# url-kaist/Quatro

Measured on NVIDIA H100. Metric: registrations/sec (64-ring pair), higher is better.
Workload: dtype f32 (front end, match, graph filter) / f64 (graph boundary, GNC, COTE)

## Files before the change

### quatro_b200/csrc/clique.cu

```cuda
#include "handle.cuh"

namespace qb {

__device__ __forceinline__ int warp_max(int v) { return __reduce_max_sync(0xffffffffu, v); }
__device__ __forceinline__ int warp_sum(int v) { return __reduce_add_sync(0xffffffffu, v); }

__device__ void warp_bucket_sort(const unsigned short* __restrict__ key, int n, int maxkey, int* __restrict__ bin,
                                 unsigned short* __restrict__ pos, unsigned short* __restrict__ vert) {
  const int lane = lane_id();
  for (int d = lane; d <= maxkey + 1; d += 32) bin[d] = 0;
  __syncwarp();
  for (int v = lane; v < n; v += 32) atomicAdd(&bin[key[v]], 1);
  __syncwarp();
  int carry = 0;
  for (int base = 0; base <= maxkey + 1; base += 32) {
    const int d = base + lane;
    const int c = d <= maxkey + 1 ? bin[d] : 0;
    int tot;
    const int ex = warp_excl_scan(c, &tot);
    if (d <= maxkey + 1) bin[d] = carry + ex;
    carry += tot;
  }
  __syncwarp();
  for (int base = 0; base < n; base += 32) {
// ... 26 lines not shown
constexpr int kRing = 16;

__device__ __forceinline__ void cp_async4(void* smem_dst, const void* gsrc) {
  const unsigned d = (unsigned)__cvta_generic_to_shared(smem_dst);
  asm volatile("cp.async.ca.shared.global [%0], [%1], 4;" ::"r"(d), "l"(gsrc) : "memory");
}
__device__ __forceinline__ void cp_async_commit() { asm volatile("cp.async.commit_group;" ::: "memory"); }
template <int N>
__device__ __forceinline__ void cp_async_wait() { asm volatile("cp.async.wait_group %0;" ::"n"(N) : "memory"); }

constexpr int kKcWarps = 4;

__device__ __forceinline__ void kcore_apply_moves(const unsigned short* __restrict__ nbl, int cnt, int dv, int* __restrict__ bin,
                                                  unsigned short* __restrict__ deg, unsigned short* __restrict__ pos,
                                                  unsigned short* __restrict__ vert, unsigned short* __restrict__ mrk,
                                                  uint32_t* __restrict__ above_own, uint32_t* __restrict__ add_next, bool classes) {
  const int lane = lane_id();
  const unsigned lt = (1u << lane) - 1u;
  for (int c0 = 0; c0 < cnt; c0 += 32) {
    const int e = c0 + lane;
    const bool act = e < cnt;
    const int u = act ? nbl[e] : 0;
    const int du = act ? deg[u] : -1 - lane;
    const unsigned grp = __match_any_sync(0xffffffffu, du);
    const int rank = __popc(grp & lt), m = __popc(grp);
    int b0 = 0, pu = 0;
    if (act) {
      b0 = bin[du];
      pu = pos[u];
      mrk[u] = (unsigned short)(rank + 1);
    }
    __syncwarp();
    int y = -1;
    if (act && pu >= b0 + m) {
      int curk = rank;
      for (;;) {
        y = vert[b0 + curk];
        const int r = mrk[y];
        if (r == 0) break;
        curk = r - 1;
      }
    }
    __syncwarp();
    if (act) {
      vert[b0 + rank] = (unsigned short)u; pos[u] = (unsigned short)(b0 + rank);
      if (y >= 0) { vert[pu] = (unsigned short)y; pos[y] = (unsigned short)pu; }
      mrk[u] = 0;
      deg[u] = (unsigned short)(du - 1);
      const uint32_t bit = 1u << (u & 31);
      if (classes) {
        atomicAnd(&above_own[u >> 5], ~bit);
        if (du - 1 > dv) atomicOr(&add_next[u >> 5], bit);
      } else if (du - 1 == dv) {
        atomicAnd(&above_own[u >> 5], ~bit);
      }
      if (rank == 0) bin[du] = b0 + m;
    }
    __syncwarp();
  }
}

template <int WPL>
__device__ __forceinline__ int kcore_expand(const uint32_t (&w)[WPL], int w0, unsigned short* __restrict__ nbl) {
  int c = 0;
#pragma unroll
  for (int k = 0; k < WPL; ++k) c += __popc(w[k]);
  int cnt;
  int off = warp_excl_scan(c, &cnt);
  if (cnt != 0) {
#pragma unroll
    for (int k = 0; k < WPL; ++k) {
      uint32_t x = w[k];
      const int basebit = (w0 + k) * 32;
      while (x) {
        const int b = __ffs(x) - 1;
        x &= x - 1;
        nbl[off++] = (unsigned short)(basebit + b);
      }
    }
  }
  return cnt;
}

template <int WPL, bool kWs>
__global__ void __maxnreg__(168) kcore_kernel(const uint32_t* __restrict__ adj, const int* __restrict__ deg_in,
                                                              const int* __restrict__ n_corr, const PairSolve* __restrict__ solve, int Lc, int W,
                                                              int Ls, int row_words, unsigned char* __restrict__ ws, int* __restrict__ kcore,
                                                              int* __restrict__ korder, int* __restrict__ rank_of, int* __restrict__ by_rank,
                                                              int* __restrict__ kbin, int* __restrict__ max_core_out) {
  constexpr int NW = kKcWarps, AW = 32 * WPL;
  extern __shared__ __align__(16) unsigned char smem_raw[];
  __shared__ int ring_tag[kRing];

  const int pair = blockIdx.x, tid = threadIdx.x, lane = tid & 31, warp = tid >> 5;
  if (solve[pair].mode == QB200_INLIER_NONE) return;
  const int L = n_corr[pair];
  if ((L > Ls) != kWs) return;
  constexpr bool in_smem = !kWs;
  const int Lv = in_smem ? Ls : Lc;
  int* bin = in_smem ? reinterpret_cast<int*>(smem_raw)
                     : reinterpret_cast<int*>(ws + (size_t)pair * kcore_ws_bytes(Lc));
  uint32_t* above = in_smem ? reinterpret_cast<uint32_t*>(bin + Ls + 2)
                            : reinterpret_cast<uint32_t*>(smem_raw);
  uint32_t* add = above + NW * AW;
  uint32_t* rows = add + 2 * NW * AW;
  unsigned short* deg = in_smem ? reinterpret_cast<unsigned short*>(rows + row_words) : reinterpret_cast<unsigned short*>(bin + Lc + 2);
  unsigned short* pos = deg + Lv;
  unsigned short* vert = pos + Lv;
  unsigned short* mrk = vert + Lv;
  unsigned short* nbl_all = mrk + Lv;
  int* __restrict__ kc = kcore + (size_t)pair * (Lc + 2);
  int* __restrict__ ko = korder + (size_t)pair * (Lc + 2);
  int* __restrict__ ro = rank_of + (size_t)pair * (Lc + 2);
  int* __restrict__ br = by_rank + (size_t)pair * (Lc + 2);
  int* __restrict__ kb = kbin + (size_t)pair * (Lc + 2);
  if (L <= 0) {
    if (tid == 0) max_core_out[pair] = 0;
    return;
  }
  const uint32_t* __restrict__ G = adj + (size_t)pair * Lc * W;
  const int nbw = (L + 31) >> 5;
  const int nwl = (nbw + 31) >> 5;
  const bool cached = in_smem && (long long)L * nbw <= (long long)row_words;
  const int rs = in_smem ? Ls / 32 : W;
  const int w0 = lane * nwl;
  unsigned short* nbl = nbl_all + (size_t)warp * Lv;

  int md = 0;
  for (int v = tid; v < L; v += NW * 32) {
    const int d = deg_in[(size_t)pair * Lc + v];
    deg[v] = (unsigned short)d;
    mrk[v] = 0;
    md = max(md, d);
  }
  if (cached)
    for (int idx = tid; idx < L * nbw; idx += NW * 32) rows[idx] = G[(size_t)(idx / nbw) * W + (idx % nbw)];
  for (int wd = tid; wd < 3 * NW * AW; wd += NW * 32) above[wd] = 0u;
  __shared__ int s_md[NW];
  md = warp_max(md);
  if (lane == 0) s_md[warp] = md;
  __syncthreads();
  md = max(max(s_md[0], s_md[1]), max(s_md[2], s_md[3]));
  if (warp == 0) warp_bucket_sort(deg, L, md, bin, pos, vert);
  __syncthreads();
  for (int v = tid; v < L; v += NW * 32) {
    const int c = cached ? 0 : (int)deg[v] % NW;
    atomicOr(&above[c * AW + (v >> 5)], 1u << (v & 31));
  }
  __syncthreads();

  int cur = -1;
  if (cached) {
    if (warp != 0) return;
    for (int i = 0; i < L; ++i) {
      const int v = vert[i];
      const int dv = deg[v];
      if (dv > cur) {
        const int end = bin[dv + 1];
        for (int p = i + lane; p < end; p += 32) {
          const int x = vert[p];
          atomicAnd(&above[x >> 5], ~(1u << (x & 31)));
        }
        cur = dv;
        __syncwarp();
      }
      uint32_t w[WPL];
#pragma unroll
      for (int k = 0; k < WPL; ++k) w[k] = (k < nwl && w0 + k < nbw) ? (rows[v * nbw + w0 + k] & above[w0 + k]) : 0u;
      const int cnt = kcore_expand<WPL>(w, w0, nbl);
      if (cnt == 0) continue;
      __syncwarp();
      kcore_apply_moves(nbl, cnt, dv, bin, deg, pos, vert, mrk, above, above, false);
    }
  } else {
    uint32_t* above_w = above + warp * AW;
    const int lower = (warp + NW - 1) % NW;
    auto fetch = [&](int p) {
      if (p < L) {
        const int x = vert[p], sl = p % kRing;
        if (lane == 0) ring_tag[sl] = x;
#pragma unroll
        for (int k = 0; k < WPL; ++k)
          if (k < nwl && w0 + k < nbw) cp_async4(rows + sl * rs + w0 + k, G + (size_t)x * W + w0 + k);
      }
      cp_async_commit();
    };
    if (warp == 0) {
      for (int p = 0; p < kRing - 1; ++p) fetch(p);
      cp_async_wait<kRing - 2>();
    }
    __syncthreads();
    for (int i = 0; i < L; ++i) {
      const int v = vert[i];
      const int dv = deg[v];
      const int par = i & 1;
      if (warp == 0) fetch(i + kRing - 1);
      uint32_t* add_in = add + ((par ^ 1) * NW + warp) * AW;
      uint32_t w[WPL];
      const int sl = i % kRing;
      const bool hit = ring_tag[sl] == v;
#pragma unroll
      for (int k = 0; k < WPL; ++k) {
        w[k] = 0u;
        if (k < nwl && w0 + k < nbw) {
          const uint32_t a = add_in[w0 + k];
          if (a) { above_w[w0 + k] |= a; add_in[w0 + k] = 0u; }
          w[k] = hit ? rows[sl * rs + w0 + k] : G[(size_t)v * W + w0 + k];
        }
      }
      __syncwarp();
      if (dv > cur) {
        if (dv % NW == warp) {
          const int end = bin[dv + 1];
          for (int p = i + lane; p < end; p += 32) {
            const int x = vert[p];
            atomicAnd(&above_w[x >> 5], ~(1u << (x & 31)));
          }
          __syncwarp();
        }
        cur = dv;
      }
#pragma unroll
      for (int k = 0; k < WPL; ++k) w[k] = (k < nwl && w0 + k < nbw) ? (w[k] & above_w[w0 + k]) : 0u;
      const int cnt = kcore_expand<WPL>(w, w0, nbl);
      if (cnt != 0) {
        __syncwarp();
        kcore_apply_moves(nbl, cnt, dv, bin, deg, pos, vert, mrk, above_w, add + (par * NW + lower) * AW, true);
      }
      if (warp == 0) cp_async_wait<kRing - 2>();
      __syncthreads();
    }
    if (warp == 0) cp_async_wait<0>();
    if (warp != 0) return;
  }
  __syncwarp();
  const int max_core = deg[vert[L - 1]];
  for (int v = lane; v < L; v += 32) {
    kc[v] = (int)deg[v] + 1;
    ko[v] = vert[v];
  }
  if (lane == 0) max_core_out[pair] = max_core;
  __syncwarp();
  warp_bucket_sort(deg, L, max_core, bin, pos, vert);
  for (int v = lane; v < L; v += 32) {
    ro[v] = pos[v];
    br[v] = vert[v];
  }
  for (int d = lane; d <= max_core + 1; d += 32) kb[d] = bin[d];
}

__global__ void __launch_bounds__(256) permute_adj_kernel(const uint32_t* __restrict__ adj, const int* __restrict__ n_corr, int Lc, int W,
                                                          const PairSolve* __restrict__ solve, const int* __restrict__ rank_of,
                                                          uint32_t* __restrict__ adjp) {
  extern __shared__ uint32_t rows[];
  const int pair = blockIdx.y;
  if (solve[pair].mode == QB200_INLIER_NONE) return;
  const int L = n_corr[pair];
  const int wib = threadIdx.x >> 5, lane = lane_id();
  const int v = blockIdx.x * 8 + wib;
  if (v >= L) return;
  uint32_t* row = rows + wib * W;
  const int nb = (L + 31) >> 5;
  for (int w = lane; w < nb; w += 32) row[w] = 0;
  __syncwarp();
  const int* __restrict__ ro = rank_of + (size_t)pair * (Lc + 2);
  const uint32_t* __restrict__ src = adj + ((size_t)pair * Lc + v) * W;
  for (int w = lane; w < nb; w += 32) {
    uint32_t x = src[w];
    while (x) {
      const int b = __ffs(x) - 1;
      x &= x - 1;
      const int r = ro[w * 32 + b];
      atomicOr(&row[r >> 5], 1u << (r & 31));
    }
  }
  __syncwarp();
  uint32_t* __restrict__ dst = adjp + ((size_t)pair * Lc + ro[v]) * W;
  for (int w = lane; w < nb; w += 32) dst[w] = row[w];
}

template <int WPL>
__device__ __forceinline__ int clique_descent(const uint32_t* __restrict__ rows, int stride, int nbw, int rv, int thr, int mc,
                                              unsigned short* __restrict__ chain) {
  const int lane = lane_id();
  uint32_t P[WPL];
  int psize = 0;
#pragma unroll
  for (int k = 0; k < WPL; ++k) {
    const int wi = lane + 32 * k;
    uint32_t x = wi < nbw ? rows[(size_t)rv * stride + wi] : 0u;
    const int lo = wi * 32;
    if (thr >= lo + 32) x = 0;
    else if (thr > lo) x &= ~0u << (thr - lo);
    P[k] = x;
    psize += __popc(x);
  }
  psize = warp_sum(psize);
  if (psize <= mc) return 0;
  int sz = 1;
  for (;;) {
    int top = -1;
#pragma unroll
    for (int k = 0; k < WPL; ++k)
      if (P[k]) top = max(top, (lane + 32 * k) * 32 + 31 - __clz(P[k]));
    top = warp_max(top);
    if (top < 0) break;
    if (lane == 0) chain[sz - 1] = (unsigned short)top;
    ++sz;
#pragma unroll
    for (int k = 0; k < WPL; ++k) {
      const int wi = lane + 32 * k;
      P[k] &= wi < nbw ? rows[(size_t)top * stride + wi] : 0u;
    }
  }
  return sz;
}

__global__ void __launch_bounds__(kCliqueWarps * 32) clique_cta_kernel(const uint32_t* __restrict__ adjp, const int* __restrict__ n_corr, int Lc, int W,
                                                                       int Ls, unsigned short* __restrict__ chain_ws,
                                                                       const int* __restrict__ kcore, const int* __restrict__ korder,
                                                                       const int* __restrict__ rank_of, const int* __restrict__ by_rank,
                                                                       const int* __restrict__ kbin, const int* __restrict__ max_core_in,
                                                                       const PairSolve* __restrict__ solve, int cache_words, int* __restrict__ clique,
                                                                       int* __restrict__ n_clique) {
  constexpr int NT = kCliqueWarps * 32;
  extern __shared__ __align__(16) unsigned char smem_raw[];
  uint32_t* idbits = reinterpret_cast<uint32_t*>(smem_raw + (size_t)kCliqueWarps * Ls * sizeof(unsigned short));
  uint32_t* cache = idbits + W;
  __shared__ int s_sz[kCliqueWarps];
  __shared__ int s_scan[33];
  const int pair = blockIdx.x, tid = threadIdx.x, lane = tid & 31, warp = tid >> 5;
// ... 196 lines not shown
      const int a = max(thr, lo), b = min(L, lo + 32);
      if (wi < nbw && a < b) x = (b - lo >= 32 ? ~0u : ((1u << (b - lo)) - 1u)) & (~0u << (a - lo));
      P[k] = x;
      if (wi < nbw) SP[wi] = x;
    }
  }
  int used = exact_colour_sort<WPL>(rows, stride, nbw, P, best, LP, kExactPool);
  bool truncated = used < 0;
  int depth = truncated ? -1 : 0;
  if (lane == 0 && !truncated) { lb[0] = 0; ln[0] = used; }
  __syncwarp();
  long long nodes = 0;
  bool improved = false;
  while (depth >= 0) {
    const int n_here = ln[depth];
    if (n_here == 0) { --depth; continue; }
    const int begin = lb[depth];
    const uint32_t e = LP[begin + n_here - 1];
    __syncwarp();
    if (lane == 0) ln[depth] = n_here - 1;
    const int v = (int)(e & 0xFFFFu), col = (int)(e >> 16);
    if (depth + col <= best) {
      if (lane == 0) ln[depth] = 0;
      __syncwarp();
      continue;
    }
    if (lane == 0) C[depth] = (unsigned short)v;
    uint32_t* __restrict__ Pl = SP + (size_t)depth * W;
    int cnt = 0;
#pragma unroll
    for (int k = 0; k < WPL; ++k) {
      const int wi = lane + 32 * k;
      uint32_t x = 0u;
      if (wi < nbw) {
        const uint32_t pw = Pl[wi];
        x = pw & rows[(size_t)v * stride + wi];
        if (wi == (v >> 5)) Pl[wi] = pw & ~(1u << (v & 31));
      }
      P[k] = x;
      cnt += __popc(x);
    }
    cnt = __reduce_add_sync(0xffffffffu, cnt);
    __syncwarp();
    if (cnt == 0) {
      if (depth + 1 > best) {
        best = depth + 1;
        improved = true;
        for (int t = lane; t <= depth; t += 32) out[t] = br[C[t]];
        __syncwarp();
        if (best >= ub) break;
      }
      continue;
    }
    if (depth + 1 + cnt <= best) continue;
    if (++nodes > node_limit || depth + 1 >= kExactDepth) { truncated = true; break; }
    const int nbegin = begin + n_here - 1;
    uint32_t* __restrict__ Pn = SP + (size_t)(depth + 1) * W;
#pragma unroll
    for (int k = 0; k < WPL; ++k) {
      const int wi = lane + 32 * k;
      if (wi < nbw) Pn[wi] = P[k];
    }
    const int nl = exact_colour_sort<WPL>(rows, stride, nbw, P, best - (depth + 1), LP + nbegin, kExactPool - nbegin);
    if (nl < 0) { truncated = true; break; }
    if (lane == 0) { lb[depth + 1] = nbegin; ln[depth + 1] = nl; }
    __syncwarp();
    ++depth;
  }
  __syncwarp();
  if (improved) {
    for (int t = lane; t < best; t += 32) {
      const int x = out[t];
      int r = 0;
      for (int u = 0; u < best; ++u) r += out[u] < x ? 1 : 0;
      lb[r] = x;
    }
    __syncwarp();
    for (int t = lane; t < best; t += 32) out[t] = lb[t];
    if (lane == 0) n_clique[pair] = best;
  }
  if (lane == 0 && truncated) flags[pair] |= QB200_FLAG_CLIQUE_TRUNCATED;
}

constexpr size_t kKcoreSmemBudget = 144 * 1024;

template <int WPL>
static int launch_kcore(Lane* h, int n_pairs) {
  const int Lc = h->Lc, W = h->W;
  const int Ls = Lc < kKcoreSmemVerts ? Lc : kKcoreSmemVerts, Ws = Ls / 32;
  const size_t bits = (size_t)3 * kKcWarps * 32 * WPL * sizeof(uint32_t);
  const size_t fixed = (size_t)(Ls + 2) * sizeof(int) + bits + (size_t)(4 + kKcWarps) * Ls * sizeof(unsigned short);
  size_t row_words = fixed + 8 * 1024 < kKcoreSmemBudget ? (kKcoreSmemBudget - fixed) / 4 : 0;
  if (row_words < (size_t)kRing * Ws) row_words = (size_t)kRing * Ws;
  if (row_words > (size_t)Ls * Ws) row_words = (size_t)Ls * Ws;
  const size_t smem = fixed + row_words * 4;
  if (Ls < Lc && smem - bits < (size_t)kRing * W * 4) {
    h->fail(__FILE__, __LINE__, "k-core prefetch ring does not fit");
    return QB200_ERR_CUDA;
  }
  QB_CUDA_TRY(h, ensure_dyn_smem(h->device, (const void*)kcore_kernel<WPL, false>, smem));
  kcore_kernel<WPL, false><<<n_pairs, kKcWarps * 32, smem, h->stream>>>(h->adj, h->deg, h->ctr.n_corr, h->d_solve, Lc, W, Ls, (int)row_words, h->kcore_ws,
                                                                        h->kcore, h->korder, h->rank_of, h->by_rank, h->kbin, h->ctr.max_core);
  if (Ls < Lc) {
    QB_CUDA_TRY(h, ensure_dyn_smem(h->device, (const void*)kcore_kernel<WPL, true>, smem));
    kcore_kernel<WPL, true><<<n_pairs, kKcWarps * 32, smem, h->stream>>>(h->adj, h->deg, h->ctr.n_corr, h->d_solve, Lc, W, Ls, (int)row_words, h->kcore_ws,
                                                                         h->kcore, h->korder, h->rank_of, h->by_rank, h->kbin, h->ctr.max_core);
    h->launches++;
  }
  return QB200_OK;
}

static int ensure_exact_scratch(Lane* h) {
  if (h->ex_stack) return QB200_OK;
  const size_t S = h->S < kExactChunk ? h->S : kExactChunk;
  DeviceMem<uint32_t> stack, pool;
  DeviceMem<int> lvl;
  DeviceMem<unsigned short> cur;
  QB_CUDA_TRY(h, stack.alloc(S * kExactDepth * (size_t)h->W));
  QB_CUDA_TRY(h, pool.alloc(S * (size_t)kExactPool));
  QB_CUDA_TRY(h, lvl.alloc(S * 2 * (size_t)kExactDepth));
  QB_CUDA_TRY(h, cur.alloc(S * (size_t)kExactDepth));
  h->ex_stack = std::move(stack);
  h->ex_pool = std::move(pool);
  h->ex_lvl = std::move(lvl);
  h->ex_cur = std::move(cur);
  return QB200_OK;
}

template <int WPL>
static int launch_exact(Lane* h, int n_pairs, int cache_words) {
  QB_CUDA_TRY(h, ensure_dyn_smem(h->device, (const void*)clique_exact_kernel<WPL>, (size_t)cache_words * 4));
  const int chunk = h->S < kExactChunk ? h->S : kExactChunk;
  for (int base = 0; base < n_pairs; base += chunk) {
    const int np = n_pairs - base < chunk ? n_pairs - base : chunk;
    clique_exact_kernel<WPL><<<np, 32, (size_t)cache_words * 4, h->stream>>>(
        h->adjp, h->ctr.n_corr, h->Lc, h->W, h->by_rank, h->rank_of, h->kbin, h->ctr.max_core, h->d_solve, cache_words, base, h->ex_stack,
        h->ex_pool, h->ex_lvl, h->ex_lvl + (size_t)chunk * kExactDepth, h->ex_cur, h->clique, h->ctr.n_clique, h->ctr.flags);
    h->launches++;
  }
  return QB200_OK;
}

int launch_clique(Lane* h, int n_pairs, bool any_exact) {
  if (n_pairs <= 0) return QB200_OK;
  const int Lc = h->Lc, W = h->W;
  const int Ls = Lc < kKcoreSmemVerts ? Lc : kKcoreSmemVerts;
  const int cache_words = 14336;
  const size_t sm_clique = (size_t)kCliqueWarps * Ls * sizeof(unsigned short) + (size_t)W * sizeof(uint32_t) + (size_t)cache_words * 4;
  int rc;
  QB_CUDA_TRY(h, ensure_dyn_smem(h->device, (const void*)clique_cta_kernel, sm_clique));
  if (any_exact && (rc = ensure_exact_scratch(h))) return rc;
  if (W <= 32) rc = launch_kcore<1>(h, n_pairs);
  else if (W <= 64) rc = launch_kcore<2>(h, n_pairs);
  else if (W <= 128) rc = launch_kcore<4>(h, n_pairs);
  else if (W <= 256) rc = launch_kcore<8>(h, n_pairs);
  else if (W <= 512) rc = launch_kcore<16>(h, n_pairs);
  else rc = launch_kcore<32>(h, n_pairs);
  if (rc) return rc;
  const dim3 gp((Lc + 7) / 8, n_pairs);
  permute_adj_kernel<<<gp, 256, 8 * W * sizeof(uint32_t), h->stream>>>(h->adj, h->ctr.n_corr, Lc, W, h->d_solve, h->rank_of, h->adjp);
  clique_cta_kernel<<<n_pairs, kCliqueWarps * 32, sm_clique, h->stream>>>(h->adjp, h->ctr.n_corr, Lc, W, Ls, h->chain_ws, h->kcore, h->korder,
                                                                          h->rank_of, h->by_rank, h->kbin, h->ctr.max_core, h->d_solve,
                                                                          cache_words, h->clique, h->ctr.n_clique);
  h->launches += 3;
  if (any_exact) {
    if (W <= 32) rc = launch_exact<1>(h, n_pairs, cache_words);
    else if (W <= 64) rc = launch_exact<2>(h, n_pairs, cache_words);
    else if (W <= 128) rc = launch_exact<4>(h, n_pairs, cache_words);
    else if (W <= 256) rc = launch_exact<8>(h, n_pairs, cache_words);
    else if (W <= 512) rc = launch_exact<16>(h, n_pairs, cache_words);
    else rc = launch_exact<32>(h, n_pairs, cache_words);
    if (rc) return rc;
  }
  QB_CUDA_TRY(h, cudaGetLastError());
  return QB200_OK;
}

}
```

### quatro_b200/csrc/handle.cuh

```cuda
#pragma once
#include <string.h>

#include <memory>
#include <vector>

#include "common.cuh"
#include "owners.cuh"

namespace qb {

struct GraphConst {
  float b2, hb2q, twob2, b4;
  float c1, c2, c3;
  float two_b2_slack;
  double beta;
};

struct PoseParams {
  double rot_noise_bound, cote_range, gnc_factor, cost_threshold;
  int max_iterations, cote_median, use_rot_inliers, use_RyRx;
  double RyRx[9];
};

struct PairSolve {
// ... 120 lines not shown
  DeviceMem<int> clique;
  DeviceMem<uint32_t> ex_stack, ex_pool;
  DeviceMem<int> ex_lvl;
  DeviceMem<unsigned short> ex_cur;
  DeviceMem<unsigned char> kcore_ws;
  DeviceMem<unsigned short> chain_ws;
  DeviceMem<unsigned char> pose_ws;
  DeviceMem<int> final_inl;
  DeviceMem<unsigned char> rot_mask, trans_mask;
  DeviceMem<PairSolve> d_solve; PinnedMem<PairSolve> h_solve;
  DeviceMem<CloudFront> d_front; PinnedMem<CloudFront> h_front;
  DeviceMem<int> pp_cnt; PinnedMem<int> pp_hcnt;
  DeviceMem<PpScan> d_pp; PinnedMem<PpScan> h_pp;
  DeviceMem<int> pw_ints;
  DeviceMem<float4> pw_out;
  int pw_scans;
  DeviceMem<void> ip_buf; size_t ip_cap;
  DeviceMem<qb200_result> d_results;
  PinnedMem<qb200_result> h_results;
  PinnedMem<unsigned char> lst_stage; int lst_cap;
  PinnedMem<unsigned char> exp_stage; size_t exp_bytes;
  WaveCounters ctr, hctr;
  DeviceMem<int> ctr_block; PinnedMem<int> hctr_block; size_t ctr_ints;

  Event ev[9];
  Event kev[4];
  int kev_armed[2];

  void fail(const char* file, int line, const char* msg) { snprintf(err, kErrLen, "%s:%d: %s", file, line, msg); }
  static constexpr int kErrLen = 512;

  size_t colpart_count() const { return (size_t)2 * S * V + (size_t)S * (V >> 7) * 2 + 2; }
  unsigned long long* colpart_col() const { return colpart; }
  unsigned long long* colpart_row() const { return colpart + (size_t)S * V; }
  unsigned* colpart_tile_cmax() const { return reinterpret_cast<unsigned*>(colpart + (size_t)2 * S * V); }
  uint32_t* class_of() const { return reinterpret_cast<uint32_t*>(key_a.get()); }
  int* n_unique() const { return reinterpret_cast<int*>(class_of() + (size_t)2 * S * V); }
};

}

struct qb200_handle {
  qb200_config cfg;
  char err[qb::Lane::kErrLen];
  std::unique_ptr<qb::Lane> lane[8];
  int max_lanes;
  int timeline;
  int lanes_active, lane_cursor;
  qb::Event ev_fork;
  qb::Stream copy_stream;
  qb::Event ev_copied;

  int c_slots;
  qb::DeviceMem<float4> c_vox, c_nrm;
  qb::DeviceMem<float> c_desc;
  qb::DeviceMem<int> c_n, c_status;
  std::unique_ptr<float[]> c_sig;

  void* comm;
  int comm_world, comm_rank, comm_cap;
  qb::Stream comm_stream;
  qb::Event comm_done;
  qb::DeviceMem<qb200_result> d_send, d_recv;
  qb::PinnedMem<qb200_result> h_send, h_recv;
  int pend_gather_n;
  qb200_result* pend_gather_dst;
  int pipe_n, pipe_buf;
  qb200_result* pipe_dst;

  double rot_noise_bound_latched;
  int last_n_corr, last_n_clique, last_n_final;
  int last_match_n[2];

  float stage_ms[8];
  float kernel_ms[2];
  int kernel_calls[2];

  void fail(const char* file, int line, const char* msg) { snprintf(err, sizeof(err), "%s:%d: %s", file, line, msg); }
};

namespace qb {

constexpr int kKcoreSmemVerts = 8192;
constexpr int kPoseSmemClique = 4096;
constexpr int kCliqueWarps = 8;
__host__ __device__ inline size_t kcore_ws_bytes(int Lc) { return ((size_t)(Lc + 2) * 4 + (size_t)8 * Lc * 2 + 15) & ~(size_t)15; }
size_t pose_ws_bytes(int Lc);

int launch_voxel(Lane* h, int n_clouds);
int launch_fpfh(Lane* h, int n_clouds);
int launch_match(Lane* h, int n_pairs, int keep_w);
int launch_match_records(Lane* h, int n_pairs);
void front_voxel(CloudFront* e, float leaf, int skip_flagged);
void front_lattice(CloudFront* e, float normal_radius, float fpfh_radius, float cell);
CloudFront front_entry(const qb200_params& p, bool lattice_only = false);
int upload_front(Lane* h, int n);
void match_fields(PairSolve* e, const qb200_params& p);
int launch_graph(Lane* h, int n_pairs);
int launch_clique(Lane* h, int n_pairs, bool any_exact);
int launch_pose(Lane* h, int n_pairs);
int launch_fill_counters(Lane* h, int n_pairs, int have_frontend);
int launch_finalize_status(Lane* h, int n_pairs);
int launch_iota_clique(Lane* h, int n_pairs);
GraphConst graph_const(double noise_bound, double cbar2);
PoseParams pose_params(const qb200_params& p);
PairSolve solve_entry(const qb200_params& p);
int upload_solve(Lane* h, int n);
struct ListDst {
  int2* corr; float4* sm; float4* tm; int* clique; int* fin; unsigned char* rm; unsigned char* tmask;
  long long stride;
  int cap;
  static ListDst caller(const qb200_pair_lists& d, long long first);
  static size_t carve(unsigned char* base, int S, int cap, const qb200_pair_lists& d, ListDst* out);
};
int launch_pack_lists(Lane* h, int n_pairs, const ListDst& dst);
__host__ __device__ inline int list_entries(int count, int Lc, int cap) {
  const int n = count < 0 ? 0 : count > Lc ? Lc : count;
  return n < cap ? n : cap;
}
int launch_match_nn(Lane* h, int n_pairs);
int launch_match_exact(Lane* h, int n_pairs, const int* only);
int launch_tc_debug_tile(Lane* h, float* d_out);
int tc_footprint(Lane* h, int* out5);
int launch_feature_export(Lane* h, int n_clouds, const ExportSrc& src, const ExportDst& dst, int max_n);
int export_desc_rows(Lane* h, const float* desc, const int* n, int m);
int stage_features(Lane* L, int n_clouds, qb200_mem_kind kind, cudaStream_t cs);
int launch_feature_import(Lane* h, int n_clouds);
size_t sort_temp_bytes(int max_items);
void comm_release(qb200_handle* h);
int collect_batch(qb200_handle* h, const qb200_result* dst);
int enter(qb200_handle* h);
bool device_array_of(const qb200_handle* h, const void* a, size_t align);
int wave_reset(Lane* L, int n_clouds);
int stage_raw(Lane* L, int ncl, qb200_mem_kind kind, cudaStream_t cs);
int launch_degree(Lane* h, int n_pairs);
int launch_row_import(Lane* h, int n_graphs, int max_L);
int launch_edge_import(Lane* h, int n_graphs, long long max_edges, int only, const int2* edges);
int launch_symmetry_check(Lane* h, int n_graphs, int max_L);
int launch_clique_records(Lane* h, int n_graphs);
bool params_ok(const qb200_params* p, bool solver = true);
float lattice_cell(const qb200_params& p);
qb200_params resolve_params(qb200_handle* h, const qb200_params& p);
void set_last(qb200_handle* h, const qb200_result& r);
cudaError_t ensure_dyn_smem(int device, const void* kernel, size_t bytes);
int sort_pairs(Lane* h, int n_items, int end_bit);
int launch_voxel_sort(Lane* h, int n_clouds, int idx_bits);
int launch_cloud_sort(Lane* h, int n_clouds, const int* n_items, int f1, int f2);

}
```

### quatro_b200/csrc/pose.cu

```cuda
#include "handle.cuh"

namespace qb {

constexpr int kPoseThreads = 256;

__device__ __forceinline__ double block_sum(double v, double* scratch) {
#pragma unroll
  for (int o = 16; o > 0; o >>= 1) v += __shfl_xor_sync(0xffffffffu, v, o);
  __syncthreads();
  if (lane_id() == 0) scratch[threadIdx.x >> 5] = v;
  __syncthreads();
  double t = 0.0;
  for (int w = 0; w < (int)(blockDim.x >> 5); ++w) t += scratch[w];
  return t;
}
__device__ __forceinline__ double block_max(double v, double* scratch) {
#pragma unroll
  for (int o = 16; o > 0; o >>= 1) v = fmax(v, __shfl_xor_sync(0xffffffffu, v, o));
  __syncthreads();
  if (lane_id() == 0) scratch[threadIdx.x >> 5] = v;
  __syncthreads();
  double t = scratch[0];
  for (int w = 1; w < (int)(blockDim.x >> 5); ++w) t = fmax(t, scratch[w]);
  return t;
}

static int next_pow2(int n) {
  int p = 32;
  while (p < n) p <<= 1;
  return p;
}
__host__ __device__ inline size_t pose_smem_bytes(int Lp) {
  return (size_t)4 * Lp * sizeof(double) + (size_t)4 * Lp * sizeof(unsigned short) + (size_t)2 * Lp;
}

__device__ void bitonic_sort(double* val, unsigned short* tag, int n2) {
  for (int k = 2; k <= n2; k <<= 1) {
    for (int j = k >> 1; j > 0; j >>= 1) {
      for (int t = threadIdx.x; t < n2; t += blockDim.x) {
        const int x = t ^ j;
        if (x > t) {
          const double a = val[t], b = val[x];
          const unsigned short ta = tag[t], tb = tag[x];
          const bool gt = (a > b) || (a == b && ta > tb);
          const bool up = (t & k) == 0;
          if (up ? gt : !gt) {
            val[t] = b; val[x] = a;
            tag[t] = tb; tag[x] = ta;
          }
        }
      }
      __syncthreads();
    }
  }
}

template <bool kWs>
__global__ void __launch_bounds__(kPoseThreads) pose_kernel(const float4* __restrict__ ma, const float4* __restrict__ mb, const int* __restrict__ n_corr,
                                                            int Lc, int Lp, int Lg, unsigned char* __restrict__ ws, const int* __restrict__ clique_all,
                                                            const int* __restrict__ n_clique, const PairSolve* __restrict__ solve,
                                                            qb200_result* __restrict__ results, unsigned char* __restrict__ rot_mask_out,
                                                            unsigned char* __restrict__ trans_mask_out, int* __restrict__ final_inl,
                                                            int* __restrict__ n_final) {
  extern __shared__ __align__(16) unsigned char smem_raw[];
  __shared__ double scratch[kPoseThreads / 32];
  __shared__ double s_bcast[4];
  __shared__ int s_ibcast[4];
  __shared__ int s_scan[33];

  const int pair = blockIdx.x, tid = threadIdx.x;
  const int L = n_corr[pair];
  const int c = n_clique[pair];
  if ((c > Lp) != kWs) return;
  const PoseParams& pp = solve[pair].pp;
  constexpr bool in_smem = !kWs;
  const int Lq = in_smem ? Lp : Lg;
  double* ev = reinterpret_cast<double*>(in_smem ? smem_raw : ws + (size_t)pair * pose_smem_bytes(Lg));
  double* wX = ev + 2 * Lq;
  double* aux = wX + Lq;
  unsigned short* tag = reinterpret_cast<unsigned short*>(aux + Lq);
  unsigned short* ctag = tag + 2 * Lq;
  unsigned short* list = ctag + Lq;
  unsigned char* rm = reinterpret_cast<unsigned char*>(list + Lq);
  unsigned char* tm = rm + Lq;
  const float4* __restrict__ A = ma + (size_t)pair * Lc;
  const float4* __restrict__ B = mb + (size_t)pair * Lc;
  const int* __restrict__ cl = clique_all + (size_t)pair * Lc;
  qb200_result* __restrict__ res = results + pair;

  if (c <= 1) {
    if (tid == 0) {
      res->valid = 0;
      res->status = (L < 2) ? QB200_DEGENERATE_INPUT : QB200_DEGENERATE_CLIQUE;
      res->clique_size = c; res->gnc_iters = 0; res->n_rot_inliers = 0; res->n_final_inliers = 0; res->cost = 0.0;
      for (int i = 0; i < 16; ++i) res->T[i] = (i % 5 == 0) ? 1.0 : 0.0;
      n_final[pair] = 0;
    }
    return;
  }

  for (int j = tid; j < c; j += kPoseThreads) wX[j] = 1.0;
  double noise_bound_sq = pp.rot_noise_bound * pp.rot_noise_bound;
  if (noise_bound_sq < 1e-16) noise_bound_sq = 1e-2;
  double mu = 1.0, prev_cost = INFINITY, cost = INFINITY;
  double r00 = 1.0, r01 = 0.0, r10 = 0.0, r11 = 1.0;
  int iters = 0;
  __syncthreads();
  for (int it = 0; it < pp.max_iterations; ++it) {
    iters = it + 1;
    double h00 = 0.0, h01 = 0.0, h10 = 0.0, h11 = 0.0;
    for (int j = tid; j < c; j += kPoseThreads) {
      const int root = cl[j], leaf = (j != c - 1) ? cl[j + 1] : cl[0];
      const float4 ar = A[root], al = A[leaf], br = B[root], bl = B[leaf];
      const double x0 = (double)al.x - (double)ar.x, x1 = (double)al.y - (double)ar.y;
      const double y0 = (double)bl.x - (double)br.x, y1 = (double)bl.y - (double)br.y;
      const double w = wX[j];
      h00 += x0 * w * y0; h01 += x0 * w * y1; h10 += x1 * w * y0; h11 += x1 * w * y1;
    }
    h00 = block_sum(h00, scratch); h01 = block_sum(h01, scratch); h10 = block_sum(h10, scratch); h11 = block_sum(h11, scratch);
    const double cc = h00 + h11, ss = h01 - h10;
    const double nn = sqrt(cc * cc + ss * ss);
    double cs = 1.0, sn = 0.0;
    if (nn > 0.0) { cs = cc / nn; sn = ss / nn; }
    r00 = cs; r01 = -sn; r10 = sn; r11 = cs;
    double mymax = -INFINITY;
    for (int j = tid; j < c; j += kPoseThreads) {
      const int root = cl[j], leaf = (j != c - 1) ? cl[j + 1] : cl[0];
      const float4 ar = A[root], al = A[leaf], br = B[root], bl = B[leaf];
      const double x0 = (double)al.x - (double)ar.x, x1 = (double)al.y - (double)ar.y;
      const double y0 = (double)bl.x - (double)br.x, y1 = (double)bl.y - (double)br.y;
      const double dx = y0 - (r00 * x0 + r01 * x1), dy = y1 - (r10 * x0 + r11 * x1);
      const double r2 = dx * dx + dy * dy;
      aux[j] = r2;
      mymax = fmax(mymax, r2);
    }
    if (it == 0) {
      const double max_residual = block_max(mymax, scratch);
      mu = 1 / (2 * max_residual / noise_bound_sq - 1);
      if (mu <= 0) break;
    }
    const double th1 = (mu + 1) / mu * noise_bound_sq;
    const double th2 = mu / (mu + 1) * noise_bound_sq;
    double pc = 0.0;
    for (int j = tid; j < c; j += kPoseThreads) {
      const double r2 = aux[j];
      pc += wX[j] * r2;
      double w;
      if (r2 >= th1) w = 0;
      else if (r2 <= th2) w = 1;
      else w = sqrt(noise_bound_sq * mu * (mu + 1) / r2) - mu;
      wX[j] = w;
    }
    cost = block_sum(pc, scratch);
    const double cost_diff = fabs(cost - prev_cost);
    mu = mu * pp.gnc_factor;
    prev_cost = cost;
// ... 105 lines not shown
  }
  __syncthreads();

  int n_fin = 0;
  {
    int carry = 0;
    for (int base = 0; base < N; base += kPoseThreads) {
      const int i = base + tid;
      const int keep = (i < N && tm[i]) ? 1 : 0;
      int tot;
      const int ex = block_excl_scan(keep, s_scan, &tot);
      if (keep) final_inl[(size_t)pair * Lc + carry + ex] = use_rot ? cl[list[i]] : cl[i];
      carry += tot;
    }
    n_fin = carry;
  }
  for (int j = tid; j < c; j += kPoseThreads) rot_mask_out[(size_t)pair * Lc + j] = rm[j];
  for (int i = tid; i < c; i += kPoseThreads) trans_mask_out[(size_t)pair * Lc + i] = i < N ? tm[i] : 0;
  if (tid == 0) {
    res->valid = 1;
    res->status = QB200_OK;
    res->clique_size = c; res->gnc_iters = iters; res->n_rot_inliers = n_rot; res->n_final_inliers = n_fin; res->cost = cost;
    double* T = res->T;
    T[0] = R[0]; T[1] = R[3]; T[2] = R[6]; T[3] = 0.0;
    T[4] = R[1]; T[5] = R[4]; T[6] = R[7]; T[7] = 0.0;
    T[8] = R[2]; T[9] = R[5]; T[10] = R[8]; T[11] = 0.0;
    T[12] = tvec[0]; T[13] = tvec[1]; T[14] = tvec[2]; T[15] = 1.0;
    n_final[pair] = n_fin;
  }
}

__global__ void fill_counters_kernel(qb200_result* __restrict__ results, int n_pairs, WaveCounters c, int have_frontend) {
  const int pair = blockIdx.x * blockDim.x + threadIdx.x;
  if (pair >= n_pairs) return;
  qb200_result* r = results + pair;
  r->n_src_vox = have_frontend ? c.n_vox[2 * pair] : 0;
  r->n_tgt_vox = have_frontend ? c.n_vox[2 * pair + 1] : 0;
  r->n_mutual = have_frontend ? c.n_mutual[pair] : 0;
  r->n_corr = c.n_corr[pair];
  r->max_core = c.max_core[pair];
  r->n_edges = c.n_edges[pair] / 2;
  r->flags = c.flags[pair];
}

__global__ void finalize_status_kernel(qb200_result* __restrict__ results, int n_pairs, WaveCounters c) {
  const int pair = blockIdx.x * blockDim.x + threadIdx.x;
  if (pair >= n_pairs) return;
  const int s0 = c.cloud_status[2 * pair], s1 = c.cloud_status[2 * pair + 1];
  const int bad = s0 != 0 ? s0 : s1;
  if (bad != 0) {
    qb200_result* r = results + pair;
    r->valid = 0;
    r->status = bad;
    for (int i = 0; i < 16; ++i) r->T[i] = (i % 5 == 0) ? 1.0 : 0.0;
  }
}

__global__ void iota_clique_kernel(const int* __restrict__ n_corr, const PairSolve* __restrict__ solve, int Lc, int* __restrict__ clique,
                                   int* __restrict__ n_clique, int* __restrict__ max_core) {
  const int pair = blockIdx.y;
  if (solve[pair].mode != QB200_INLIER_NONE) return;
  const int L = n_corr[pair];
  const int i = blockIdx.x * blockDim.x + threadIdx.x;
  if (i < L) clique[(size_t)pair * Lc + i] = i;
  if (i == 0) { n_clique[pair] = L; max_core[pair] = 0; }
}

size_t pose_ws_bytes(int Lc) { return pose_smem_bytes(next_pow2(Lc)); }

PoseParams pose_params(const qb200_params& p) {
  PoseParams pp;
  pp.rot_noise_bound = p.rot_noise_bound;
  pp.cote_range = p.cote_noise_bound * sqrt(p.cbar2);
  pp.gnc_factor = p.rotation_gnc_factor;
  pp.cost_threshold = p.rotation_cost_threshold;
  pp.max_iterations = p.rotation_max_iterations;
  pp.cote_median = p.cote_mode == QB200_COTE_MEDIAN;
  pp.use_rot_inliers = p.using_rot_inliers_when_estimating_cote;
  pp.use_RyRx = p.use_pre_estimated_RyRx;
  for (int i = 0; i < 9; ++i) pp.RyRx[i] = p.RyRx[i];
  return pp;
}

int launch_pose(Lane* h, int n_pairs) {
  if (n_pairs <= 0) return QB200_OK;
  const int Lp = next_pow2(h->Lc < kPoseSmemClique ? h->Lc : kPoseSmemClique);
  const size_t smem = pose_smem_bytes(Lp);
  QB_CUDA_TRY(h, ensure_dyn_smem(h->device, (const void*)pose_kernel<false>, smem));
  pose_kernel<false><<<n_pairs, kPoseThreads, smem, h->stream>>>(h->ma, h->mb, h->ctr.n_corr, h->Lc, Lp, next_pow2(h->Lc), h->pose_ws, h->clique,
                                                                 h->ctr.n_clique, h->d_solve, h->d_results, h->rot_mask, h->trans_mask, h->final_inl,
                                                                 h->ctr.n_final);
  h->launches++;
  if (h->Lc > kPoseSmemClique) {
    pose_kernel<true><<<n_pairs, kPoseThreads, 0, h->stream>>>(h->ma, h->mb, h->ctr.n_corr, h->Lc, Lp, next_pow2(h->Lc), h->pose_ws, h->clique,
                                                               h->ctr.n_clique, h->d_solve, h->d_results, h->rot_mask, h->trans_mask, h->final_inl,
                                                               h->ctr.n_final);
    h->launches++;
  }
  QB_CUDA_TRY(h, cudaGetLastError());
  return QB200_OK;
}

int launch_fill_counters(Lane* h, int n_pairs, int have_frontend) {
  fill_counters_kernel<<<(n_pairs + 127) / 128, 128, 0, h->stream>>>(h->d_results, n_pairs, h->ctr, have_frontend);
  h->launches++;
  return QB200_OK;
}
int launch_finalize_status(Lane* h, int n_pairs) {
  finalize_status_kernel<<<(n_pairs + 127) / 128, 128, 0, h->stream>>>(h->d_results, n_pairs, h->ctr);
  h->launches++;
  return QB200_OK;
}
int launch_iota_clique(Lane* h, int n_pairs) {
  const dim3 g((h->Lc + 255) / 256, n_pairs);
  iota_clique_kernel<<<g, 256, 0, h->stream>>>(h->ctr.n_corr, h->d_solve, h->Lc, h->clique, h->ctr.n_clique, h->ctr.max_core);
  h->launches++;
  return QB200_OK;
}

}
```

Before: 14220.

## Pack small k-core graphs four per CTA and split pose launches by clique size

Adds a packed k-core kernel in which each warp handles one pair. Small graphs share a 120 KB shared-memory arena, so several pairs run per block instead of one pair holding a mostly idle 4-warp CTA. The cached single-warp path of the main k-core kernel is factored into a reusable device function, and the main kernel now skips pairs already handled by the packed kernel. The pose stage launches a small-shared-memory variant first for cliques up to 256, then a larger one for the rest, to raise occupancy. The k-core and pose smem budgets are also lowered, at the cost of extra launches and a per-warp prefix computation of arena offsets.

```diff
diff --git a/quatro_b200/csrc/clique.cu b/quatro_b200/csrc/clique.cu
--- a/quatro_b200/csrc/clique.cu
+++ b/quatro_b200/csrc/clique.cu
@@ -132,6 +132,120 @@
   return cnt;
 }
 
+__device__ void kcore_outputs(int L, int* __restrict__ bin, unsigned short* __restrict__ deg, unsigned short* __restrict__ pos,
+                              unsigned short* __restrict__ vert, int* __restrict__ kc, int* __restrict__ ko, int* __restrict__ ro,
+                              int* __restrict__ br, int* __restrict__ kb, int* __restrict__ max_core_out) {
+  const int lane = lane_id();
+  const int max_core = deg[vert[L - 1]];
+  for (int v = lane; v < L; v += 32) {
+    kc[v] = (int)deg[v] + 1;
+    ko[v] = vert[v];
+  }
+  if (lane == 0) *max_core_out = max_core;
+  __syncwarp();
+  warp_bucket_sort(deg, L, max_core, bin, pos, vert);
+  for (int v = lane; v < L; v += 32) {
+    ro[v] = pos[v];
+    br[v] = vert[v];
+  }
+  for (int d = lane; d <= max_core + 1; d += 32) kb[d] = bin[d];
+}
+
+template <int WPL>
+__device__ void kcore_warp(const uint32_t* __restrict__ G, const int* __restrict__ dg, int L, int W, int* __restrict__ bin,
+                           uint32_t* __restrict__ above, uint32_t* __restrict__ rows, unsigned short* __restrict__ deg,
+                           unsigned short* __restrict__ pos, unsigned short* __restrict__ vert, unsigned short* __restrict__ mrk,
+                           unsigned short* __restrict__ nbl, int* __restrict__ kc, int* __restrict__ ko, int* __restrict__ ro,
+                           int* __restrict__ br, int* __restrict__ kb, int* __restrict__ max_core_out) {
+  const int lane = lane_id();
+  const int nbw = (L + 31) >> 5;
+  const int nwl = (nbw + 31) >> 5;
+  const int w0 = lane * nwl;
+  int md = 0;
+  for (int v = lane; v < L; v += 32) {
+    const int d = dg[v];
+    deg[v] = (unsigned short)d;
+    mrk[v] = 0;
+    md = max(md, d);
+  }
+  for (int idx = lane; idx < L * nbw; idx += 32) rows[idx] = G[(size_t)(idx / nbw) * W + (idx % nbw)];
+  for (int wd = lane; wd < nbw; wd += 32) above[wd] = 0u;
+  md = warp_max(md);
+  __syncwarp();
+  warp_bucket_sort(deg, L, md, bin, pos, vert);
+  for (int v = lane; v < L; v += 32) atomicOr(&above[v >> 5], 1u << (v & 31));
+  __syncwarp();
+
+  int cur = -1;
+  for (int i = 0; i < L; ++i) {
+    const int v = vert[i];
+    const int dv = deg[v];
+    if (dv > cur) {
+      const int end = bin[dv + 1];
+      for (int p = i + lane; p < end; p += 32) {
+        const int x = vert[p];
+        atomicAnd(&above[x >> 5], ~(1u << (x & 31)));
+      }
+      cur = dv;
+      __syncwarp();
+    }
+    uint32_t w[WPL];
+#pragma unroll
+    for (int k = 0; k < WPL; ++k) w[k] = (k < nwl && w0 + k < nbw) ? (rows[v * nbw + w0 + k] & above[w0 + k]) : 0u;
+    const int cnt = kcore_expand<WPL>(w, w0, nbl);
+    if (cnt == 0) continue;
+    __syncwarp();
+    kcore_apply_moves(nbl, cnt, dv, bin, deg, pos, vert, mrk, above, above, false);
+  }
+  __syncwarp();
+  kcore_outputs(L, bin, deg, pos, vert, kc, ko, ro, br, kb, max_core_out);
+}
+
+constexpr int kKcPackWarps = 4;
+constexpr int kKcArenaBytes = 120 * 1024;
+__host__ __device__ constexpr int kcore_carve_bytes(int L) {
+  return L <= 0 ? 0 : ((L + 2) * 4 + ((L + 31) >> 5) * (1 + L) * 4 + 10 * L + 15) & ~15;
+}
+static_assert(kcore_carve_bytes(1024) > kKcArenaBytes, "a packed graph has at most 32 adjacency words per row: one per lane");
+
+__device__ __forceinline__ int kcore_packed_offset(int pair, const int* __restrict__ n_corr, const PairSolve* __restrict__ solve) {
+  int off = 0;
+  for (int q = pair - pair % kKcPackWarps; q <= pair; ++q) {
+    if (solve[q].mode == QB200_INLIER_NONE) continue;
+    const int b = kcore_carve_bytes(n_corr[q]);
+    const bool fits = off + b <= kKcArenaBytes;
+    if (q == pair) return fits ? off : -1;
+    if (fits) off += b;
+  }
+  return -1;
+}
+
+__global__ void __launch_bounds__(kKcPackWarps * 32) kcore_packed_kernel(const uint32_t* __restrict__ adj, const int* __restrict__ deg_in,
+                                                                         const int* __restrict__ n_corr, const PairSolve* __restrict__ solve,
+                                                                         int n_pairs, int Lc, int W, int* __restrict__ kcore,
+                                                                         int* __restrict__ korder, int* __restrict__ rank_of,
+                                                                         int* __restrict__ by_rank, int* __restrict__ kbin,
+                                                                         int* __restrict__ max_core_out) {
+  extern __shared__ __align__(16) unsigned char smem_raw[];
+  const int warp = threadIdx.x >> 5, pair = blockIdx.x * kKcPackWarps + warp;
+  if (pair >= n_pairs || solve[pair].mode == QB200_INLIER_NONE) return;
+  const int L = n_corr[pair];
+  const int off = kcore_packed_offset(pair, n_corr, solve);
+  if (off < 0) return;
+  if (L <= 0) {
+    if (lane_id() == 0) max_core_out[pair] = 0;
+    return;
+  }
+  const int nbw = (L + 31) >> 5;
+  int* bin = reinterpret_cast<int*>(smem_raw + off);
+  uint32_t* above = reinterpret_cast<uint32_t*>(bin + L + 2);
+  uint32_t* rows = above + nbw;
+  unsigned short* deg = reinterpret_cast<unsigned short*>(rows + (size_t)L * nbw);
+  const size_t o = (size_t)pair * (Lc + 2);
+  kcore_warp<1>(adj + (size_t)pair * Lc * W, deg_in + (size_t)pair * Lc, L, W, bin, above, rows, deg, deg + L, deg + 2 * L, deg + 3 * L,
+                deg + 4 * L, kcore + o, korder + o, rank_of + o, by_rank + o, kbin + o, max_core_out + pair);
+}
+
 template <int WPL, bool kWs>
 __global__ void __maxnreg__(168) kcore_kernel(const uint32_t* __restrict__ adj, const int* __restrict__ deg_in,
                                                               const int* __restrict__ n_corr, const PairSolve* __restrict__ solve, int Lc, int W,
@@ -145,6 +259,7 @@
   const int pair = blockIdx.x, tid = threadIdx.x, lane = tid & 31, warp = tid >> 5;
   if (solve[pair].mode == QB200_INLIER_NONE) return;
   const int L = n_corr[pair];
+  if (kcore_packed_offset(pair, n_corr, solve) >= 0) return;
   if ((L > Ls) != kWs) return;
   constexpr bool in_smem = !kWs;
   const int Lv = in_smem ? Ls : Lc;
@@ -164,14 +279,14 @@
   int* __restrict__ ro = rank_of + (size_t)pair * (Lc + 2);
   int* __restrict__ br = by_rank + (size_t)pair * (Lc + 2);
   int* __restrict__ kb = kbin + (size_t)pair * (Lc + 2);
-  if (L <= 0) {
-    if (tid == 0) max_core_out[pair] = 0;
-    return;
-  }
   const uint32_t* __restrict__ G = adj + (size_t)pair * Lc * W;
   const int nbw = (L + 31) >> 5;
   const int nwl = (nbw + 31) >> 5;
-  const bool cached = in_smem && (long long)L * nbw <= (long long)row_words;
+  if (in_smem && (long long)L * nbw <= (long long)row_words) {
+    if (warp == 0) kcore_warp<WPL>(G, deg_in + (size_t)pair * Lc, L, W, bin, above, rows, deg, pos, vert, mrk, nbl_all, kc, ko, ro, br, kb,
+                                   max_core_out + pair);
+    return;
+  }
   const int rs = in_smem ? Ls / 32 : W;
   const int w0 = lane * nwl;
   unsigned short* nbl = nbl_all + (size_t)warp * Lv;
@@ -183,8 +298,6 @@
     mrk[v] = 0;
     md = max(md, d);
   }
-  if (cached)
-    for (int idx = tid; idx < L * nbw; idx += NW * 32) rows[idx] = G[(size_t)(idx / nbw) * W + (idx % nbw)];
   for (int wd = tid; wd < 3 * NW * AW; wd += NW * 32) above[wd] = 0u;
   __shared__ int s_md[NW];
   md = warp_max(md);
@@ -194,35 +307,13 @@
   if (warp == 0) warp_bucket_sort(deg, L, md, bin, pos, vert);
   __syncthreads();
   for (int v = tid; v < L; v += NW * 32) {
-    const int c = cached ? 0 : (int)deg[v] % NW;
+    const int c = (int)deg[v] % NW;
     atomicOr(&above[c * AW + (v >> 5)], 1u << (v & 31));
   }
   __syncthreads();
 
   int cur = -1;
-  if (cached) {
-    if (warp != 0) return;
-    for (int i = 0; i < L; ++i) {
-      const int v = vert[i];
-      const int dv = deg[v];
-      if (dv > cur) {
-        const int end = bin[dv + 1];
-        for (int p = i + lane; p < end; p += 32) {
-          const int x = vert[p];
-          atomicAnd(&above[x >> 5], ~(1u << (x & 31)));
-        }
-        cur = dv;
-        __syncwarp();
-      }
-      uint32_t w[WPL];
-#pragma unroll
-      for (int k = 0; k < WPL; ++k) w[k] = (k < nwl && w0 + k < nbw) ? (rows[v * nbw + w0 + k] & above[w0 + k]) : 0u;
-      const int cnt = kcore_expand<WPL>(w, w0, nbl);
-      if (cnt == 0) continue;
-      __syncwarp();
-      kcore_apply_moves(nbl, cnt, dv, bin, deg, pos, vert, mrk, above, above, false);
-    }
-  } else {
+  {
     uint32_t* above_w = above + warp * AW;
     const int lower = (warp + NW - 1) % NW;
     auto fetch = [&](int p) {
@@ -284,19 +375,7 @@
     if (warp != 0) return;
   }
   __syncwarp();
-  const int max_core = deg[vert[L - 1]];
-  for (int v = lane; v < L; v += 32) {
-    kc[v] = (int)deg[v] + 1;
-    ko[v] = vert[v];
-  }
-  if (lane == 0) max_core_out[pair] = max_core;
-  __syncwarp();
-  warp_bucket_sort(deg, L, max_core, bin, pos, vert);
-  for (int v = lane; v < L; v += 32) {
-    ro[v] = pos[v];
-    br[v] = vert[v];
-  }
-  for (int d = lane; d <= max_core + 1; d += 32) kb[d] = bin[d];
+  kcore_outputs(L, bin, deg, pos, vert, kc, ko, ro, br, kb, max_core_out + pair);
 }
 
 __global__ void __launch_bounds__(256) permute_adj_kernel(const uint32_t* __restrict__ adj, const int* __restrict__ n_corr, int Lc, int W,
@@ -659,7 +738,7 @@
   if (lane == 0 && truncated) flags[pair] |= QB200_FLAG_CLIQUE_TRUNCATED;
 }
 
-constexpr size_t kKcoreSmemBudget = 144 * 1024;
+constexpr size_t kKcoreSmemBudget = 120 * 1024;
 
 template <int WPL>
 static int launch_kcore(Lane* h, int n_pairs) {
@@ -727,6 +806,11 @@
   int rc;
   QB_CUDA_TRY(h, ensure_dyn_smem(h->device, (const void*)clique_cta_kernel, sm_clique));
   if (any_exact && (rc = ensure_exact_scratch(h))) return rc;
+  const size_t sm_packed = kKcArenaBytes;
+  QB_CUDA_TRY(h, ensure_dyn_smem(h->device, (const void*)kcore_packed_kernel, sm_packed));
+  kcore_packed_kernel<<<(n_pairs + kKcPackWarps - 1) / kKcPackWarps, kKcPackWarps * 32, sm_packed, h->stream>>>(
+      h->adj, h->deg, h->ctr.n_corr, h->d_solve, n_pairs, Lc, W, h->kcore, h->korder, h->rank_of, h->by_rank, h->kbin, h->ctr.max_core);
+  h->launches++;
   if (W <= 32) rc = launch_kcore<1>(h, n_pairs);
   else if (W <= 64) rc = launch_kcore<2>(h, n_pairs);
   else if (W <= 128) rc = launch_kcore<4>(h, n_pairs);
diff --git a/quatro_b200/csrc/handle.cuh b/quatro_b200/csrc/handle.cuh
--- a/quatro_b200/csrc/handle.cuh
+++ b/quatro_b200/csrc/handle.cuh
@@ -226,7 +226,7 @@
 namespace qb {
 
 constexpr int kKcoreSmemVerts = 8192;
-constexpr int kPoseSmemClique = 4096;
+constexpr int kPoseSmemClique = 2048;
 constexpr int kCliqueWarps = 8;
 __host__ __device__ inline size_t kcore_ws_bytes(int Lc) { return ((size_t)(Lc + 2) * 4 + (size_t)8 * Lc * 2 + 15) & ~(size_t)15; }
 size_t pose_ws_bytes(int Lc);
diff --git a/quatro_b200/csrc/pose.cu b/quatro_b200/csrc/pose.cu
--- a/quatro_b200/csrc/pose.cu
+++ b/quatro_b200/csrc/pose.cu
@@ -57,7 +57,7 @@
 
 template <bool kWs>
 __global__ void __launch_bounds__(kPoseThreads) pose_kernel(const float4* __restrict__ ma, const float4* __restrict__ mb, const int* __restrict__ n_corr,
-                                                            int Lc, int Lp, int Lg, unsigned char* __restrict__ ws, const int* __restrict__ clique_all,
+                                                            int Lc, int Lp, int c_below, int Lg, unsigned char* __restrict__ ws, const int* __restrict__ clique_all,
                                                             const int* __restrict__ n_clique, const PairSolve* __restrict__ solve,
                                                             qb200_result* __restrict__ results, unsigned char* __restrict__ rot_mask_out,
                                                             unsigned char* __restrict__ trans_mask_out, int* __restrict__ final_inl,
@@ -71,7 +71,7 @@
   const int pair = blockIdx.x, tid = threadIdx.x;
   const int L = n_corr[pair];
   const int c = n_clique[pair];
-  if ((c > Lp) != kWs) return;
+  if ((c > Lp) != kWs || c <= c_below) return;
   const PoseParams& pp = solve[pair].pp;
   constexpr bool in_smem = !kWs;
   const int Lq = in_smem ? Lp : Lg;
@@ -343,17 +343,23 @@
   return pp;
 }
 
+constexpr int kPoseSmallClique = 256;
+
 int launch_pose(Lane* h, int n_pairs) {
   if (n_pairs <= 0) return QB200_OK;
   const int Lp = next_pow2(h->Lc < kPoseSmemClique ? h->Lc : kPoseSmemClique);
-  const size_t smem = pose_smem_bytes(Lp);
-  QB_CUDA_TRY(h, ensure_dyn_smem(h->device, (const void*)pose_kernel<false>, smem));
-  pose_kernel<false><<<n_pairs, kPoseThreads, smem, h->stream>>>(h->ma, h->mb, h->ctr.n_corr, h->Lc, Lp, next_pow2(h->Lc), h->pose_ws, h->clique,
-                                                                 h->ctr.n_clique, h->d_solve, h->d_results, h->rot_mask, h->trans_mask, h->final_inl,
-                                                                 h->ctr.n_final);
-  h->launches++;
+  const int Lps = Lp < kPoseSmallClique ? Lp : kPoseSmallClique;
+  QB_CUDA_TRY(h, ensure_dyn_smem(h->device, (const void*)pose_kernel<false>, pose_smem_bytes(Lp)));
+  auto launch_smem = [&](int lp, int below) {
+    pose_kernel<false><<<n_pairs, kPoseThreads, pose_smem_bytes(lp), h->stream>>>(h->ma, h->mb, h->ctr.n_corr, h->Lc, lp, below, next_pow2(h->Lc),
+                                                                                 h->pose_ws, h->clique, h->ctr.n_clique, h->d_solve, h->d_results,
+                                                                                 h->rot_mask, h->trans_mask, h->final_inl, h->ctr.n_final);
+    h->launches++;
+  };
+  launch_smem(Lps, -1);
+  if (Lp > Lps) launch_smem(Lp, Lps);
   if (h->Lc > kPoseSmemClique) {
-    pose_kernel<true><<<n_pairs, kPoseThreads, 0, h->stream>>>(h->ma, h->mb, h->ctr.n_corr, h->Lc, Lp, next_pow2(h->Lc), h->pose_ws, h->clique,
+    pose_kernel<true><<<n_pairs, kPoseThreads, 0, h->stream>>>(h->ma, h->mb, h->ctr.n_corr, h->Lc, Lp, -1, next_pow2(h->Lc), h->pose_ws, h->clique,
                                                                h->ctr.n_clique, h->d_solve, h->d_results, h->rot_mask, h->trans_mask, h->final_inl,
                                                                h->ctr.n_final);
     h->launches++;
```

Result: faster. 14500 (median of 6 runs) (+2.0%).
